# apache/auron

Measured on AMD Instinct MI355X. Metric: tpcds_suite_seconds, lower is better.
Workload: dtype decimal64/fp64

## Files before the change

auron_amd/config.py:

```python
from __future__ import annotations

import os
from dataclasses import dataclass
from typing import Any, Dict, Optional


@dataclass(frozen=True)
class ConfigOption:
    key: str
    default: Any
    typ: type
    doc: str = ""
    env: Optional[str] = None


_REGISTRY: Dict[str, ConfigOption] = {}


def _opt(key: str, default, typ, doc="", env=None) -> ConfigOption:
    o = ConfigOption(key, default, typ, doc, env)
    _REGISTRY[key] = o
    return o


BATCH_SIZE = _opt("spark.auron.batchSize", 1 << 22, int, "rows per in-flight batch")
MEMORY_FRACTION = _opt("spark.auron.memoryFraction", 0.8, float, "fraction of HBM the memmgr may use")
ENABLE_NATIVE = _opt("spark.auron.enable", True, bool, "master switch")
REQUIRE_NATIVE = _opt("spark.auron.requireNativeKernels", True, bool,
                      "fail loudly if HIP kernels missing on GPU", env="AURON_REQUIRE_NATIVE")
SPILL_COMPRESSION = _opt("spark.auron.spill.compression.codec", "lz4", str)
SHUFFLE_COMPRESSION = _opt("spark.auron.shuffle.compression.codec", "none", str,
                           "xGMI is fast enough that intra-node shuffle ships raw")
SMJ_FALLBACK_ENABLE = _opt("spark.auron.smjfallback.enable", False, bool, env="AURON_SMJ_FALLBACK")
SMJ_FALLBACK_ROWS = _opt("spark.auron.smjfallback.rows.threshold", 10_000_000, int, env="AURON_SMJ_FALLBACK_ROWS")
PARTIAL_AGG_SKIPPING_RATIO = _opt("spark.auron.partialAggSkipping.ratio", 0.999, float, env="AURON_PARTIAL_SKIP_RATIO")
UDF_FALLBACK = _opt("spark.auron.udf.hostFallback.enable", True, bool)
LOG_LEVEL = _opt("spark.auron.native.log.level", "WARN", str, env="AURON_LOG_LEVEL")
IGNORE_CORRUPTED_FILES = _opt("spark.auron.ignoreCorruptedFiles", False, bool,
                              "skip unreadable input files instead of failing the task",
                              env="AURON_IGNORE_CORRUPTED_FILES")
BROADCAST_MAX_ROWS = _opt("spark.auron.broadcast.maxRows", 20_000_000, int,
                          "estimated build-side rows above which the planner "
                          "shuffles both join sides instead of broadcasting",
                          env="AURON_BROADCAST_MAX_ROWS")
BROADCAST_CACHE_BYTES = _opt("spark.auron.broadcast.cache.maxBytes", 4 << 30, int,
                             "device bytes of build-once broadcast relations/"
                             "hash tables kept across queries",
                             env="AURON_BROADCAST_CACHE_BYTES")
FORCE_SHUFFLED_HASH_JOIN = _opt("spark.auron.forceShuffledHashJoin", False, bool,
                                "never broadcast: hash-exchange both sides",
                                env="AURON_FORCE_SHJ")
EXPR_FUSION = _opt("spark.auron.expr.fusion.enable", False, bool,
                   "compile project/filter scalar expression trees into one "
                   "fused interpreter kernel launch (k_expr_exec). Default "
                   "off: the kernel itself measures ~24us/launch but the "
                   "per-batch host dispatch costs more than the at::native "
                   "launches it replaces at TPC-DS shapes (same-box A/B: "
                   "SF=10 suite 8.24s on vs 6.52s off); worthwhile only for "
                   "very wide scalar-heavy projections until the native "
                   "plan walker absorbs the dispatch",
                   env="AURON_EXPR_FUSION")
AGG_STREAMING = _opt("spark.auron.agg.streaming.enable", True, bool,
                     "chunked spill-capable partial aggregation",
                     env="AURON_AGG_STREAMING")
HOST_SPILL_BUDGET = _opt("spark.auron.memory.hostSpillBudget", 64 << 30, int,
                         "host-DRAM bytes of spilled holders before the disk "
                         "tier engages", env="AURON_HOST_SPILL_BUDGET")
SHUFFLE_PERSIST = _opt("spark.auron.shuffle.persist", False, bool,
                       "route exchanges through durable .data/.index files "
                       "(stage-retry contract)", env="AURON_SHUFFLE_PERSIST")
PARQUET_NATIVE = _opt("spark.auron.parquet.native.enable", True, bool,
                      "device parquet decode (else pyarrow host read)",
                      env="AURON_PARQUET_NATIVE")
PARQUET_PAGE_DECOMPRESS = _opt("spark.auron.parquet.pageDecompression.enable",
                               True, bool,
                               "host-decompress snappy/zstd/gzip pages for "
                               "the device decode path")
PARTIAL_AGG_SKIPPING_MINROWS = _opt("spark.auron.partialAggSkipping.minRows",
                                    1 << 14, int,
                                    "below this many rows partial-agg "
                                    "skipping is never sampled")
SORT_LIMIT_TOPK = _opt("spark.auron.sort.topK.enable", True, bool,
                       "ORDER BY+LIMIT keeps only the top K rows per batch")
SORT_EXTERNAL_WIDE_KEYS = _opt("spark.auron.sort.external.wideKeys.enable",
                               True, bool,
                               "range-split external sort also for string and "
                               "decimal128 first keys (off: such sorts stay "
                               "monolithic and cannot spill)",
                               env="AURON_SORT_EXTERNAL_WIDE_KEYS")
EXCHANGE_SAMPLE_ROWS = _opt("spark.auron.rangePartition.sampleRows", 4096, int,
                            "per-rank sample size for range-partition bounds")
SCAN_CACHE_BYTES = _opt("spark.auron.scan.cache.maxBytes", 0, int,
                        "per-query decoded-scan cache budget; 0 = auto "
                        "(15% of HBM on GPU, 4 GB on CPU)",
                        env="AURON_SCAN_CACHE_BYTES")
STREAM_BYTES = _opt("spark.auron.stream.minInputBytes", -1, int,
                    "estimated agg-input bytes above which operators "
                    "stream instead of materializing; -1 = auto (8% of "
                    "HBM on GPU, 1 GB on CPU), 0 = always stream",
                    env="AURON_STREAM_BYTES")
SCAN_HBM_CACHE = _opt("spark.auron.scan.hbmStagedCache.maxBytes", 0, int,
                      "staged raw-page bytes kept device-resident across "
                      "reads; 0 = auto (30% of HBM)",
                      env="AURON_SCAN_HBM_CACHE")
HBM_CACHE_RESERVE = _opt("spark.auron.scan.hbmStagedCache.reserveFraction",
                         0.25, float,
                         "free-HBM fraction the staged-bytes cache must "
                         "never consume (evicts itself under pressure)")
SCAN_DELTA_NATIVE = _opt("spark.auron.scan.deltaNative.enable", True, bool,
                         "decode DELTA_BINARY_PACKED pages and "
                         "DELTA_LENGTH_BYTE_ARRAY / DELTA_BYTE_ARRAY string "
                         "pages with the k_pq_delta_* kernels from a "
                         "host-built miniblock index, DELTA_BYTE_ARRAY "
                         "strings rebuilt by k_pq_dba_bytes (off: "
                         "DELTA_BINARY_PACKED is expanded to PLAIN by one "
                         "host job per page and DELTA_LENGTH_BYTE_ARRAY and "
                         "DELTA_BYTE_ARRAY columns take the pyarrow host "
                         "read)",
                         env="AURON_SCAN_DELTA_NATIVE")
SCAN_PREFETCH = _opt("spark.auron.scan.streamPrefetch", 2, int,
                     "files decoded ahead of the consumer on the "
                     "streaming scan path")
SCAN_IO_THREADS = _opt("spark.auron.scan.ioThreads", 8, int,
                       "host page-read/staging thread-pool size",
                       env="AURON_SCAN_IO_THREADS")
STREAM_PEEK_FACTOR = _opt("spark.auron.stream.peekBatches", 8, int,
                          "batch-size multiples buffered before the "
                          "chunked agg commits to streaming")
STREAM_JOIN_PROBE = _opt("spark.auron.stream.joinProbe.enable", True, bool,
                         "probe build-right joins batch-by-batch on the "
                         "streaming path (GPU only)",
                         env="AURON_STREAM_JOIN_PROBE")
JOIN_FUSED_PROBE = _opt("spark.auron.join.fusedProbe.enable", True, bool,
                        "probe hash joins with the fused kernels "
                        "(k_join_probe_count / k_join_probe_fill / "
                        "k_join_exists: probe hash computed in-kernel, one "
                        "chain walk, per-tile offsets, key descriptors passed "
                        "by value) for up to 8 key columns (off: murmur3 + "
                        "k_join_count + torch scan + k_join_fill, and "
                        "join_counts for semi/anti/existence joins)",
                        env="AURON_JOIN_FUSED_PROBE")
DECIMAL128_NATIVE_ARITH = _opt("spark.auron.decimal128.nativeArith.enable",
                               True, bool,
                               "run exact decimal128 + - * /, comparisons, "
                               "casts, abs and CheckOverflow on the "
                               "k_dec128_* kernels (off: the exact "
                               "host-integer reference path, also on GPU "
                               "batches)",
                               env="AURON_DECIMAL128_NATIVE_ARITH")
SPILL_DIR = _opt("spark.auron.spill.dir", "", str,
                 "directory for disk-tier spill files (empty = system tmp)",
                 env="AURON_SPILL_DIR")
MEM_BUDGET = _opt("spark.auron.memory.budgetBytes", 0, int,
                  "absolute memmgr budget override; 0 = memoryFraction "
                  "of device/host memory", env="AURON_MEM_BUDGET")


class AuronConf:
    def __init__(self, overrides: Optional[Dict[str, Any]] = None):
        self._values: Dict[str, Any] = {}
        if overrides:
            for k, v in overrides.items():
                self.set(k, v)

    def set(self, key: str, value) -> "AuronConf":
        if key not in _REGISTRY:
            raise KeyError(f"unknown config {key}; known: {sorted(_REGISTRY)}")
        self._values[key] = value
        return self

    def get(self, opt: ConfigOption):
        if opt.key in self._values:
            return self._values[opt.key]
        if opt.env and opt.env in os.environ:
            raw = os.environ[opt.env]
            if opt.typ is bool:
                return raw not in ("0", "false", "False")
            return opt.typ(raw)
        return opt.default

    @staticmethod
    def options() -> Dict[str, ConfigOption]:
        return dict(_REGISTRY)
```

auron_amd/native/__init__.py:

```python
from __future__ import annotations

import ctypes
import os
from typing import List, Optional, Tuple

import numpy as np
import torch

_LIB_NAME = "libauron_hip.so"
_here = os.path.dirname(os.path.abspath(__file__))
LIB_PATH = os.path.join(_here, _LIB_NAME)

_lib = None
_load_error: Optional[str] = None


class AuronNativeMissing(RuntimeError):
    pass


def _try_load():
    global _lib, _load_error
    if _lib is not None or _load_error is not None:
        return
    if not os.path.exists(LIB_PATH):
        _load_error = f"{LIB_PATH} not built (run python -m auron_amd.native.build)"
        return
    try:
        lib = ctypes.CDLL(LIB_PATH)
    except OSError as e:
        _load_error = str(e)
        return
    c = ctypes.c_void_p
    i32 = ctypes.c_int32
    i64 = ctypes.c_int64
    lib.au_abi_version.restype = ctypes.c_int
    lib.au_murmur3.argtypes = [c, ctypes.c_int, i64, i32, c, c]
    lib.au_group_ids.argtypes = [c, ctypes.c_int, i64, c, i64, c, c, c, c, c, c]
    lib.au_join_build.argtypes = [i64, c, i64, c, c, c]
    lib.au_join_count.argtypes = [c, c, ctypes.c_int, i64, c, i64, c, c, c, c]
    lib.au_join_fill.argtypes = [c, c, ctypes.c_int, i64, c, i64, c, c, c, c, c, c, ctypes.c_int, c]
    lib.au_join_probe_tile.argtypes = []
    lib.au_join_probe_tile.restype = i64
    lib.au_join_probe_max_keys.argtypes = []
    lib.au_join_probe_max_keys.restype = ctypes.c_int
    lib.au_join_probe_count.argtypes = [c, ctypes.c_int, i64, c, i64, c, i32,
                                        ctypes.c_int, c, c, c, c, c]
    lib.au_join_probe_fill.argtypes = [c, ctypes.c_int, i64, c, c, c, c,
                                       ctypes.c_int, c, c, c]
    lib.au_join_exists.argtypes = [c, ctypes.c_int, i64, c, i64, c, i32, c, c]
    for f in ("au_join_probe_count", "au_join_probe_fill", "au_join_exists"):
        getattr(lib, f).restype = ctypes.c_int
    lib.au_pmod.argtypes = [c, i64, i32, c, c]
    lib.au_bytes_gather.argtypes = [c, c, c, c, i64, c]
    lib.au_multi_gather.argtypes = [c, i64, c, ctypes.c_int, c]
    lib.au_multi_gather.restype = ctypes.c_int
    lib.au_agg_scatter.argtypes = [c, i64, c, c, ctypes.c_int, ctypes.c_int,
                                   ctypes.c_int, c, c, i64, c]
    lib.au_agg_count.argtypes = [c, i64, c, c, c]
    lib.au_agg_multi.argtypes = [c, i64, c, ctypes.c_int, c]
    for f in ("au_agg_scatter", "au_agg_count", "au_agg_multi"):
        getattr(lib, f).restype = ctypes.c_int
    lib.au_pq_rle1.argtypes = [c, ctypes.c_int, c, c, c]
    lib.au_rle1_expand.argtypes = [c, i64, c, c, c]
    lib.au_rle1_expand.restype = ctypes.c_int
    lib.au_host_rle1_parse.argtypes = [c, i64, i64, i64, i64, c, i64]
    lib.au_host_rle1_parse.restype = i64
    lib.au_host_plainba_parse.argtypes = [c, i64, i64, c, c, i64]
    lib.au_host_plainba_parse.restype = i64
    lib.au_host_delta_unpack.argtypes = [c, i64, i64, i64, ctypes.c_int, c]
    lib.au_host_delta_unpack.restype = i64
    lib.au_host_delta_index.argtypes = [c, i64, i64, i64, i64, i64, i64, c, c,
                                        i64]
    lib.au_host_delta_index.restype = i64
    lib.au_pq_delta_sums.argtypes = [c, i64, c, c, c]
    lib.au_pq_delta_scan.argtypes = [c, i64, c]
    lib.au_pq_delta_emit.argtypes = [c, i64, c, i64, c, c, c, ctypes.c_int, c]
    for f in ("au_pq_delta_sums", "au_pq_delta_scan", "au_pq_delta_emit"):
        getattr(lib, f).restype = ctypes.c_int
    lib.au_host_dba_decode.argtypes = [c, i64, c, c, c, c, i64, c, i64]
    lib.au_host_dba_decode.restype = i64
    lib.au_pq_dba_tile.argtypes = []
    lib.au_pq_dba_tile.restype = i64
    lib.au_pq_dba_bytes.argtypes = [c, c, c, c, i64, i64, c, c, c]
    lib.au_pq_dba_bytes.restype = ctypes.c_int
    lib.au_pq_rle_idx.argtypes = [c, ctypes.c_int, c, c, c, c]
    lib.au_pq_scatter.argtypes = [c, ctypes.c_int, c, c, c, c, ctypes.c_int, i64, c]
    lib.au_pq_copy_plain.argtypes = [c, ctypes.c_int, c, c, ctypes.c_int, i64, c]
    for f in ("au_pq_rle1", "au_pq_rle_idx", "au_pq_scatter", "au_pq_copy_plain"):
        getattr(lib, f).restype = ctypes.c_int
    lib.au_expr_exec.argtypes = [c, ctypes.c_int, c, ctypes.c_int, c,
                                 ctypes.c_int, ctypes.c_int, i64, c]
    lib.au_expr_exec.restype = ctypes.c_int
    lib.au_part_hist.argtypes = [c, i64, i32, c, c]
    lib.au_part_scatter.argtypes = [c, i64, c, c, c, c]
    lib.au_range_bucket_str.argtypes = [c, c, i64, c, c, i32, ctypes.c_int, c, c]
    lib.au_range_bucket_i128.argtypes = [c, i64, c, i32, ctypes.c_int, c, c]
    for f in ("au_range_bucket_str", "au_range_bucket_i128"):
        getattr(lib, f).restype = ctypes.c_int
    f64 = ctypes.c_double
    lib.au_window_range_bounds_i64.argtypes = [c, c, c, i64, i64, i64,
                                               ctypes.c_int, c, c, c]
    lib.au_window_range_bounds_f64.argtypes = [c, c, c, i64, f64, f64,
                                               ctypes.c_int, c, c, c]
    lib.au_window_frame_minmax_i64.argtypes = [c, i64, c, i64, c, c, i64,
                                               ctypes.c_int, c, c]
    lib.au_window_frame_minmax_f64.argtypes = [c, i64, c, i64, c, c, i64,
                                               ctypes.c_int, c, c]
    lib.au_window_pyramid_size.argtypes = [i64]
    lib.au_window_pyramid_size.restype = i64
    lib.au_i128_scan_tile.argtypes = []
    lib.au_i128_scan_tile.restype = i64
    lib.au_prefix_sum_i128.argtypes = [c, c, i64, c, c, c]
    lib.au_window_frame_sum_i128.argtypes = [c, i64, c, c, i64, c, c]
    lib.au_window_frame_minmax_i128.argtypes = [c, i64, c, i64, c, c, i64,
                                                ctypes.c_int, c, c]
    for f in ("au_window_range_bounds_i64", "au_window_range_bounds_f64",
              "au_window_frame_minmax_i64", "au_window_frame_minmax_f64",
              "au_prefix_sum_i128", "au_window_frame_sum_i128",
              "au_window_frame_minmax_i128"):
        getattr(lib, f).restype = ctypes.c_int
    ci = ctypes.c_int
    u64 = ctypes.c_uint64
    lib.au_dec128_grid_threads.argtypes = []
    lib.au_dec128_grid_threads.restype = i64
    lib.au_dec128_addsub.argtypes = [c, ci, c, c, ci, c, i64, ci, ci, ci, ci,
                                     ci, c, c, c]
    lib.au_dec128_mul.argtypes = [c, ci, c, c, ci, c, i64, ci, ci, c, c, c]
    lib.au_dec128_div.argtypes = [c, ci, c, c, ci, c, i64, ci, ci, c, c, c]
    lib.au_dec128_cmp.argtypes = [c, ci, c, ci, i64, ci, ci, ci, c, c]
    lib.au_dec128_rescale.argtypes = [c, ci, c, i64, ci, ci, u64, u64, c, ci,
                                      c, c]
    for f in ("au_dec128_addsub", "au_dec128_mul", "au_dec128_div",
              "au_dec128_cmp", "au_dec128_rescale"):
        getattr(lib, f).restype = ctypes.c_int
    for f in ("au_murmur3", "au_group_ids", "au_join_build", "au_join_count",
              "au_join_fill", "au_pmod", "au_part_hist", "au_part_scatter"):
        getattr(lib, f).restype = ctypes.c_int
    _lib = lib


def available() -> bool:
    _try_load()
    return _lib is not None


def require():
    _try_load()
    if _lib is None:
        raise AuronNativeMissing(
            f"auron native HIP library unavailable: {_load_error}. "
            "Build it with `python -m auron_amd.native.build`."
        )
    return _lib


def lib():
    return require()


def host_lib():
    return require()


_DESC_DTYPE = np.dtype(
    [("data", "<u8"), ("offsets", "<u8"), ("validity", "<u8"),
     ("dtype", "<i4"), ("scale", "<i4")]
)
assert _DESC_DTYPE.itemsize == 32


def pack_descs_host(cols) -> Tuple[np.ndarray, list]:
    n = len(cols)
    arr = np.zeros(n, dtype=_DESC_DTYPE)
    keep = []
    for i, col in enumerate(cols):
        data = col.data
        if not data.is_contiguous():
            data = data.contiguous()
        if col.dtype.code == 12 and data.data_ptr() % 16:
            raise ValueError("decimal128 key column is not 16-byte aligned "
                             "(ops._key_cols aligns it)")
        keep.append(data)
        arr[i]["data"] = data.data_ptr()
        if col.offsets is not None:
            off = col.offsets.contiguous()
            keep.append(off)
            arr[i]["offsets"] = off.data_ptr()
        if col.validity is not None:
            v = col.validity.contiguous()
            keep.append(v)
# ... 25 lines not shown
```

auron_amd/native/csrc/kernels.hip:

```cpp

#include <hip/hip_runtime.h>
#include <stdint.h>

#define AU_EXPORT extern "C" __attribute__((visibility("default")))

enum AuDType : int32_t {
  AU_BOOL = 0,
  AU_INT8 = 1,
  AU_INT16 = 2,
  AU_INT32 = 3,
  AU_INT64 = 4,
  AU_FLOAT32 = 5,
  AU_FLOAT64 = 6,
  AU_DATE32 = 7,
  AU_STRING = 8,
  AU_DECIMAL64 = 9,
  AU_LIST = 10,
  AU_TIMESTAMP = 11,
  AU_DECIMAL128 = 12,
};

struct AuColDesc {
  const void* data;
  const int64_t* offsets;
// ... 120 lines not shown
      return hash_bytes((const uint8_t*)c.data + s, (int32_t)(e - s), seed);
    }
    case AU_DECIMAL128: {
      const ulonglong2 v = ((const ulonglong2*)c.data)[i];
      return hash_dec128(v.x, (int64_t)v.y, seed);
    }
  }
  return seed;
}

__global__ void k_murmur3(const AuColDesc* cols, int ncols, int64_t n,
                          uint32_t seed, int32_t* out) {
  for (int64_t i = (int64_t)blockIdx.x * blockDim.x + threadIdx.x; i < n;
       i += (int64_t)gridDim.x * blockDim.x) {
    uint32_t h = seed;
    for (int c = 0; c < ncols; c++) {
      if (row_valid(cols[c], i)) h = hash_one(cols[c], i, h);
    }
    out[i] = (int32_t)h;
  }
}

AU_EXPORT int au_murmur3(const void* cols_dev, int ncols, int64_t n,
                         int32_t seed, int32_t* out, void* stream) {
  if (n == 0) return 0;
  hipLaunchKernelGGL(k_murmur3, dim3(au_grid(n, 256)), dim3(256), 0,
                     (hipStream_t)stream, (const AuColDesc*)cols_dev, ncols, n,
                     (uint32_t)seed, out);
  return (int)hipGetLastError();
}

__device__ bool keys_equal(const AuColDesc* a_cols, int64_t ai,
                           const AuColDesc* b_cols, int64_t bi, int ncols) {
  for (int c = 0; c < ncols; c++) {
    const AuColDesc& a = a_cols[c];
    const AuColDesc& b = b_cols[c];
    bool av = row_valid(a, ai);
    bool bv = row_valid(b, bi);
    if (av != bv) return false;
    if (!av) continue;
    switch (a.dtype) {
      case AU_BOOL:
      case AU_INT8:
        if (((const int8_t*)a.data)[ai] != ((const int8_t*)b.data)[bi]) return false;
        break;
      case AU_INT16:
        if (((const int16_t*)a.data)[ai] != ((const int16_t*)b.data)[bi]) return false;
        break;
      case AU_INT32:
      case AU_DATE32:
        if (((const int32_t*)a.data)[ai] != ((const int32_t*)b.data)[bi]) return false;
        break;
      case AU_INT64:
      case AU_DECIMAL64:
      case AU_TIMESTAMP:
        if (((const int64_t*)a.data)[ai] != ((const int64_t*)b.data)[bi]) return false;
        break;
      case AU_FLOAT32:
        if (((const float*)a.data)[ai] != ((const float*)b.data)[bi]) return false;
        break;
      case AU_FLOAT64:
        if (((const double*)a.data)[ai] != ((const double*)b.data)[bi]) return false;
        break;
      case AU_STRING: {
        int64_t as = a.offsets[ai], ae = a.offsets[ai + 1];
        int64_t bs = b.offsets[bi], be = b.offsets[bi + 1];
        if (ae - as != be - bs) return false;
        const uint8_t* ap = (const uint8_t*)a.data + as;
        const uint8_t* bp = (const uint8_t*)b.data + bs;
        int32_t len = (int32_t)(ae - as);
        int32_t k = 0;
        for (; k + 8 <= len; k += 8) {
          uint64_t wa, wb;
          __builtin_memcpy(&wa, ap + k, 8);
          __builtin_memcpy(&wb, bp + k, 8);
          if (wa != wb) return false;
        }
        for (; k < len; k++)
          if (ap[k] != bp[k]) return false;
        break;
      }
      case AU_DECIMAL128: {
        const ulonglong2 va = ((const ulonglong2*)a.data)[ai];
        const ulonglong2 vb = ((const ulonglong2*)b.data)[bi];
        if (va.x != vb.x || va.y != vb.y) return false;
        break;
      }
    }
  }
  return true;
}

__global__ void k_group_insert(const AuColDesc* cols, int ncols, int64_t n,
                               int32_t* slots, uint32_t cap_mask,
                               const int32_t* hashes, int32_t* rep) {
  for (int64_t i = (int64_t)blockIdx.x * blockDim.x + threadIdx.x; i < n;
       i += (int64_t)gridDim.x * blockDim.x) {
    uint32_t p = ((uint32_t)hashes[i]) & cap_mask;
    int32_t me = (int32_t)i;
    while (true) {
      int32_t cur = slots[p];
      if (cur == -1) {
        int32_t prev = atomicCAS(&slots[p], -1, me);
        if (prev == -1) {
          rep[i] = me;
          break;
        }
        cur = prev;
      }
      if (keys_equal(cols, cur, cols, i, ncols)) {
        rep[i] = cur;
        break;
      }
      p = (p + 1) & cap_mask;
    }
  }
}

__global__ void k_group_assign(const int32_t* rep, int64_t n, int32_t* gid_of_row,
                               int64_t* rep_rows, int32_t* counter) {
  for (int64_t i = (int64_t)blockIdx.x * blockDim.x + threadIdx.x; i < n;
       i += (int64_t)gridDim.x * blockDim.x) {
    if (rep[i] == (int32_t)i) {
      int32_t g = atomicAdd(counter, 1);
      gid_of_row[i] = g;
      rep_rows[g] = i;
    }
  }
}

__global__ void k_group_gather(const int32_t* rep, int64_t n, int32_t* gid_of_row) {
  for (int64_t i = (int64_t)blockIdx.x * blockDim.x + threadIdx.x; i < n;
       i += (int64_t)gridDim.x * blockDim.x) {
    gid_of_row[i] = gid_of_row[rep[i]];
  }
}

AU_EXPORT int au_group_ids(const void* cols_dev, int ncols, int64_t n,
                           int32_t* slots, int64_t cap, const int32_t* hashes,
                           int32_t* rep, int32_t* gids, int64_t* rep_rows,
                           int32_t* counter, void* stream) {
  if (n == 0) return 0;
  hipStream_t s = (hipStream_t)stream;
  uint32_t mask = (uint32_t)(cap - 1);
  int g = au_grid(n, 256);
  hipLaunchKernelGGL(k_group_insert, dim3(g), dim3(256), 0, s,
                     (const AuColDesc*)cols_dev, ncols, n, slots, mask, hashes, rep);
  hipLaunchKernelGGL(k_group_assign, dim3(g), dim3(256), 0, s, rep, n, gids,
                     rep_rows, counter);
  hipLaunchKernelGGL(k_group_gather, dim3(g), dim3(256), 0, s, rep, n, gids);
  return (int)hipGetLastError();
}

__global__ void k_join_build(int64_t n, int32_t* heads, uint32_t cap_mask,
                             int32_t* next, const int32_t* hashes) {
  for (int64_t i = (int64_t)blockIdx.x * blockDim.x + threadIdx.x; i < n;
       i += (int64_t)gridDim.x * blockDim.x) {
    uint32_t p = ((uint32_t)hashes[i]) & cap_mask;
    next[i] = atomicExch(&heads[p], (int32_t)i);
  }
}

__device__ __forceinline__ bool join_row_has_null(const AuColDesc* cols,
                                                  int ncols, int64_t i) {
  for (int c = 0; c < ncols; c++)
    if (!row_valid(cols[c], i)) return true;
  return false;
}

__global__ void k_join_count(const AuColDesc* bcols, const AuColDesc* pcols,
                             int ncols, int64_t n_probe, const int32_t* heads,
                             uint32_t cap_mask, const int32_t* next,
                             const int32_t* phashes, int32_t* counts) {
  for (int64_t i = (int64_t)blockIdx.x * blockDim.x + threadIdx.x; i < n_probe;
       i += (int64_t)gridDim.x * blockDim.x) {
    int32_t cnt = 0;
    if (!join_row_has_null(pcols, ncols, i)) {
      int32_t j = heads[((uint32_t)phashes[i]) & cap_mask];
      while (j != -1) {
        if (keys_equal(bcols, j, pcols, i, ncols) &&
            !join_row_has_null(bcols, ncols, j))
          cnt++;
        j = next[j];
      }
    }
    counts[i] = cnt;
  }
}

__global__ void k_join_fill(const AuColDesc* bcols, const AuColDesc* pcols,
                            int ncols, int64_t n_probe, const int32_t* heads,
                            uint32_t cap_mask, const int32_t* next,
                            const int32_t* phashes, const int64_t* offsets,
                            int64_t* build_out, int64_t* probe_out,
                            uint8_t* build_matched, int emit_unmatched_probe) {
  for (int64_t i = (int64_t)blockIdx.x * blockDim.x + threadIdx.x; i < n_probe;
       i += (int64_t)gridDim.x * blockDim.x) {
    int64_t o = offsets[i];
    int64_t start = o;
    if (!join_row_has_null(pcols, ncols, i)) {
      int32_t j = heads[((uint32_t)phashes[i]) & cap_mask];
      while (j != -1) {
        if (keys_equal(bcols, j, pcols, i, ncols) &&
            !join_row_has_null(bcols, ncols, j)) {
          build_out[o] = j;
          probe_out[o] = i;
          if (build_matched) build_matched[j] = 1;
          o++;
        }
        j = next[j];
      }
    }
    if (emit_unmatched_probe && o == start) {
      build_out[o] = -1;
      probe_out[o] = i;
    }
  }
}

AU_EXPORT int au_join_build(int64_t n, int32_t* heads, int64_t cap,
                            int32_t* next, const int32_t* hashes, void* stream) {
  if (n == 0) return 0;
  hipLaunchKernelGGL(k_join_build, dim3(au_grid(n, 256)), dim3(256), 0,
                     (hipStream_t)stream, n, heads, (uint32_t)(cap - 1), next,
                     hashes);
  return (int)hipGetLastError();
}

AU_EXPORT int au_join_count(const void* bcols, const void* pcols, int ncols,
                            int64_t n_probe, const int32_t* heads, int64_t cap,
                            const int32_t* next, const int32_t* phashes,
                            int32_t* counts, void* stream) {
  if (n_probe == 0) return 0;
  hipLaunchKernelGGL(k_join_count, dim3(au_grid(n_probe, 256)), dim3(256), 0,
                     (hipStream_t)stream, (const AuColDesc*)bcols,
                     (const AuColDesc*)pcols, ncols, n_probe, heads,
                     (uint32_t)(cap - 1), next, phashes, counts);
  return (int)hipGetLastError();
}

AU_EXPORT int au_join_fill(const void* bcols, const void* pcols, int ncols,
                           int64_t n_probe, const int32_t* heads, int64_t cap,
                           const int32_t* next, const int32_t* phashes,
                           const int64_t* offsets, int64_t* build_out,
                           int64_t* probe_out, uint8_t* build_matched,
                           int emit_unmatched_probe, void* stream) {
  if (n_probe == 0) return 0;
  hipLaunchKernelGGL(k_join_fill, dim3(au_grid(n_probe, 256)), dim3(256), 0,
                     (hipStream_t)stream, (const AuColDesc*)bcols,
                     (const AuColDesc*)pcols, ncols, n_probe, heads,
                     (uint32_t)(cap - 1), next, phashes, offsets, build_out,
                     probe_out, build_matched, emit_unmatched_probe);
  return (int)hipGetLastError();
}

#define JP_MAX_KEYS 8
#define JP_BLOCK 256
#define JP_SLABS 4
#define JP_TILE (JP_BLOCK * JP_SLABS)

struct JpKeys {
  AuColDesc build[JP_MAX_KEYS];
  AuColDesc probe[JP_MAX_KEYS];
};

template <int MODE>
__device__ __forceinline__ bool jp_probe_key(const JpKeys& k, int ncols,
                                             int64_t i, int64_t* pkey) {
  if (MODE == 0) return !join_row_has_null(k.probe, ncols, i);
  const uint8_t* v = k.probe[0].validity;
  if (v != nullptr && v[i] == 0) return false;
  if (MODE == 1) *pkey = ((const int64_t*)k.probe[0].data)[i];
  else *pkey = ((const int32_t*)k.probe[0].data)[i];
  return true;
}

template <int MODE>
__device__ __forceinline__ uint32_t jp_hash(const JpKeys& k, int ncols,
                                            int64_t i, int64_t pkey,
                                            uint32_t seed) {
  if (MODE == 1) return hash_long((uint64_t)pkey, seed);
  if (MODE == 2) return hash_int((uint32_t)(int32_t)pkey, seed);
  uint32_t h = seed;
  for (int c = 0; c < ncols; c++) h = hash_one(k.probe[c], i, h);
  return h;
}

template <int MODE>
__device__ __forceinline__ bool jp_match(const JpKeys& k, int ncols, int32_t j,
                                         int64_t i, int64_t pkey) {
  if (MODE == 0)
    return keys_equal(k.build, j, k.probe, i, ncols) &&
           !join_row_has_null(k.build, ncols, j);
  const uint8_t* v = k.build[0].validity;
  if (MODE == 1) {
    if (((const int64_t*)k.build[0].data)[j] != pkey) return false;
  } else {
    if (((const int32_t*)k.build[0].data)[j] != (int32_t)pkey) return false;
  }
  return v == nullptr || v[j] != 0;
}

template <int MODE>
__global__ void __launch_bounds__(JP_BLOCK) k_join_probe_count(
    JpKeys k, int ncols, int64_t n_probe, int64_t n_tiles,
    const int32_t* __restrict__ heads, uint32_t cap_mask,
// ... 364 lines not shown
```

auron_amd/ops.py:

```python
from __future__ import annotations

import os
from typing import List, Optional, Tuple

import torch

from . import dtypes, native
from .column import Column

SPARK_SEED = 42
_M32 = 0xFFFFFFFF
_M64 = (1 << 64) - 1


def _use_native(device: torch.device) -> bool:
    if device.type != "cuda":
        return False
    if os.environ.get("AURON_FORCE_REF", "0") == "1":
        return False
    if os.environ.get("AURON_REQUIRE_NATIVE", "1") == "0" and not native.available():
        return False
    native.require()
    return True

# ... 68 lines not shown
    idx = skip[:, None] + torch.arange(16, device=d.device)[None, :]
    return _hash_padded_bytes_t(B.gather(1, idx.clamp(max=15)), lens, 16, h)


def _spark_narrow_decimal(dt) -> bool:
    return dt.code == dtypes.DECIMAL128 and dt.precision <= 18


def murmur3_ref(cols: List[Column], seed: int = SPARK_SEED) -> torch.Tensor:
    n = len(cols[0])
    device = cols[0].device
    h = torch.full((n,), seed, dtype=torch.int64, device=device)
    for c in cols:
        if c.dtype.is_string:
            from . import strings as S

            lens = S.lengths(c)
            maxlen = int(lens.max().item()) if n else 0
            padded = S.to_padded(c, max(maxlen, 1)).to(torch.int64)
            hv = _hash_padded_bytes_t(padded, lens, maxlen, h)
        else:
            d = c.data
            code = c.dtype.code
            if code in (dtypes.BOOL,):
                v = d.to(torch.int64)
                hv = _hash_int_t(v, h)
            elif code in (dtypes.INT8, dtypes.INT16, dtypes.INT32, dtypes.DATE32):
                v = d.to(torch.int64) & _M32
                hv = _hash_int_t(v, h)
            elif code in (dtypes.INT64, dtypes.DECIMAL64):
                v = d.to(torch.int64)
                hv = _hash_long_t(v, h)
            elif code == dtypes.FLOAT32:
                f = torch.where(d == 0, torch.zeros_like(d), d)
                v = f.view(torch.int32).to(torch.int64) & _M32
                hv = _hash_int_t(v, h)
            elif code == dtypes.FLOAT64:
                f = torch.where(d == 0, torch.zeros_like(d), d)
                v = f.view(torch.int64)
                hv = _hash_long_t(v, h)
            elif code == dtypes.DECIMAL128:
                if _spark_narrow_decimal(c.dtype):
                    hv = _hash_long_t(d[:, 0], h)
                else:
                    hv = _hash_dec128_t(d, h)
            else:
                raise TypeError(c.dtype.name)
        if c.validity is not None:
            h = torch.where(c.validity, hv, h)
        else:
            h = hv
    h = torch.where(h >= 2 ** 31, h - 2 ** 32, h)
    return h.to(torch.int32)


def _key_cols(cols: List[Column]) -> List[Column]:
    out = []
    for c in cols:
        if c.dtype.code == dtypes.DECIMAL128:
            d = _i128_aligned(c.data)
            if d is not c.data:
                c = Column(c.dtype, d, c.validity)
        out.append(c)
    return out


def _spark_hash_cols(cols: List[Column]) -> List[Column]:
    out = []
    for c in cols:
        if _spark_narrow_decimal(c.dtype):
            c = Column(dtypes.decimal64(c.dtype.precision, c.dtype.scale),
                       c.data[:, 0].contiguous(), c.validity)
        out.append(c)
    return out


def _murmur3_native(cols: List[Column], seed: int = SPARK_SEED) -> torch.Tensor:
    device = cols[0].device
    n = len(cols[0])
    lib = native.lib()
    out = torch.empty(n, dtype=torch.int32, device=device)
    descs, keep = native.pack_descs(_key_cols(cols), device)
    rc = lib.au_murmur3(descs.data_ptr(), len(cols), n, seed, out.data_ptr(),
                        native.stream_ptr(device))
    native.check(rc, "au_murmur3")
    del keep
    return out


def murmur3(cols: List[Column], seed: int = SPARK_SEED) -> torch.Tensor:
    device = cols[0].device
    if not _use_native(device):
        return murmur3_ref(cols, seed)
    return _murmur3_native(_spark_hash_cols(cols), seed)


def _join_hash(cols: List[Column]) -> torch.Tensor:
    return _murmur3_native(cols)


def _next_pow2(x: int) -> int:
    p = 1024
    while p < x:
        p <<= 1
    return p


def _key_tuple_lists(cols: List[Column]):
    import math

    lists = []
    for c in cols:
        if c.dtype.code == dtypes.DECIMAL128:
            d = c.data.to("cpu")
            valid = None if c.validity is None else c.validity.tolist()
            vals = [(h << 64) | (l & _M64) for l, h in
                    zip(d[:, 0].tolist(), d[:, 1].tolist())]
            if valid is not None:
                vals = [v if ok else None for v, ok in zip(vals, valid)]
            lists.append(vals)
            continue
        vals = c.to_pylist()
        if c.dtype.is_float:
            vals = ["NaN" if (v is not None and isinstance(v, float) and math.isnan(v)) else v for v in vals]
        lists.append(vals)
    return list(zip(*lists)) if cols else []


def group_ids_ref(cols: List[Column]) -> Tuple[torch.Tensor, torch.Tensor]:
    keys = _key_tuple_lists(cols)
    d = {}
    gids = []
    reps = []
    for i, k in enumerate(keys):
        g = d.get(k)
        if g is None:
            g = len(d)
            d[k] = g
            reps.append(i)
        gids.append(g)
    device = cols[0].device
    return (torch.tensor(gids, dtype=torch.int64, device=device),
            torch.tensor(reps, dtype=torch.int64, device=device))


def group_ids(cols: List[Column]) -> Tuple[torch.Tensor, torch.Tensor]:
    device = cols[0].device
    n = len(cols[0])
    if n == 0:
        return (torch.empty(0, dtype=torch.int64, device=device),
                torch.empty(0, dtype=torch.int64, device=device))
    if not _use_native(device):
        return group_ids_ref(cols)
    lib = native.lib()
    cols = _key_cols(cols)
    hashes = murmur3(cols)
    cap = _next_pow2(2 * n)
    slots = torch.full((cap,), -1, dtype=torch.int32, device=device)
    rep = torch.empty(n, dtype=torch.int32, device=device)
    gids = torch.empty(n, dtype=torch.int32, device=device)
    rep_rows = torch.empty(n, dtype=torch.int64, device=device)
    counter = torch.zeros(1, dtype=torch.int32, device=device)
    descs, keep = native.pack_descs(cols, device)
    rc = lib.au_group_ids(descs.data_ptr(), len(cols), n, slots.data_ptr(), cap,
                          hashes.data_ptr(), rep.data_ptr(), gids.data_ptr(),
                          rep_rows.data_ptr(), counter.data_ptr(),
                          native.stream_ptr(device))
    native.check(rc, "au_group_ids")
    ng = int(counter.item())
    del keep
    return gids.to(torch.int64), rep_rows[:ng]


def hash_join_ref(build_cols, probe_cols, emit_unmatched_probe, need_build_matched):
    bkeys = _key_tuple_lists(build_cols)
    pkeys = _key_tuple_lists(probe_cols)
    table = {}
    for j, k in enumerate(bkeys):
        if any(v is None for v in k):
            continue
        table.setdefault(k, []).append(j)
    n_build = len(build_cols[0]) if build_cols else 0
    matched = [False] * n_build
    bi, pi = [], []
    for i, k in enumerate(pkeys):
        rows = [] if any(v is None for v in k) else table.get(k, [])
        if rows:
            for j in rows:
                bi.append(j)
                pi.append(i)
                matched[j] = True
        elif emit_unmatched_probe:
            bi.append(-1)
            pi.append(i)
    device = probe_cols[0].device
    bm = torch.tensor(matched, dtype=torch.bool, device=device) if need_build_matched else None
    return (torch.tensor(bi, dtype=torch.int64, device=device),
            torch.tensor(pi, dtype=torch.int64, device=device), bm)



class JoinTable:

    __slots__ = ("heads", "nxt", "cap", "bhash", "n_build")

    def __init__(self, heads, nxt, cap, bhash, n_build):
        self.heads = heads
        self.nxt = nxt
        self.cap = cap
        self.bhash = bhash
        self.n_build = n_build

    @property
    def nbytes(self):
        return (self.heads.numel() + self.nxt.numel()) * 4 + self.bhash.numel() * 8


def join_build(build_cols: List[Column]) -> Optional["JoinTable"]:
    device = build_cols[0].device
    if not _use_native(device):
        return None
    lib = native.lib()
    sp = native.stream_ptr(device)
    n_build = len(build_cols[0])
    bhash = _join_hash(build_cols)
    cap = _next_pow2(2 * max(n_build, 1))
    heads = torch.full((cap,), -1, dtype=torch.int32, device=device)
    nxt = torch.empty(max(n_build, 1), dtype=torch.int32, device=device)
    if n_build:
        rc = lib.au_join_build(n_build, heads.data_ptr(), cap, nxt.data_ptr(),
                               bhash.data_ptr(), sp)
        native.check(rc, "au_join_build")
    return JoinTable(heads, nxt, cap, bhash, n_build)


JOIN_PROBE_MAX_KEYS = 8


def _fused_probe_enabled() -> bool:
    from .config import JOIN_FUSED_PROBE, AuronConf

    return bool(AuronConf().get(JOIN_FUSED_PROBE))


def join_probe_tile() -> int:
    return int(native.lib().au_join_probe_tile())


def _join_key_descs(build_cols, probe_cols):
    import numpy as np

    barr, bkeep = native.pack_descs_host(_key_cols(build_cols))
    parr, pkeep = native.pack_descs_host(_key_cols(probe_cols))
    return np.concatenate([barr, parr]), (bkeep, pkeep)


def hash_join(build_cols: List[Column], probe_cols: List[Column],
              emit_unmatched_probe: bool = False,
              need_build_matched: bool = False,
              table: Optional["JoinTable"] = None):
    device = probe_cols[0].device
    n_probe = len(probe_cols[0])
    n_build = len(build_cols[0])
    if not _use_native(device):
        return hash_join_ref(build_cols, probe_cols, emit_unmatched_probe, need_build_matched)
    if table is None:
        table = join_build(build_cols)
    if len(build_cols) <= JOIN_PROBE_MAX_KEYS and _fused_probe_enabled():
        return _hash_join_fused(build_cols, probe_cols, emit_unmatched_probe,
                                need_build_matched, table)
    return _hash_join_legacy(build_cols, probe_cols, emit_unmatched_probe,
                             need_build_matched, table)


def _hash_join_fused(build_cols, probe_cols, emit_unmatched_probe,
                     need_build_matched, table):
    device = probe_cols[0].device
    n_probe = len(probe_cols[0])
    n_build = len(build_cols[0])
    lib = native.lib()
    sp = native.stream_ptr(device)
    bm = torch.zeros(n_build, dtype=torch.uint8, device=device) if need_build_matched else None
    if n_probe == 0:
        empty = torch.empty(0, dtype=torch.int64, device=device)
        return empty, empty.clone(), (bm.bool() if bm is not None else None)
    ncols = len(build_cols)
    descs, keep = _join_key_descs(build_cols, probe_cols)
    tile = join_probe_tile()
    n_tiles = (n_probe + tile - 1) // tile
    counts = torch.empty(n_probe, dtype=torch.int32, device=device)
    first = torch.empty(n_probe, dtype=torch.int32, device=device)
    tile_sums = torch.empty(n_tiles, dtype=torch.int64, device=device)
    emit = 1 if emit_unmatched_probe else 0
    rc = lib.au_join_probe_count(descs.ctypes.data, ncols, n_probe,
                                 table.heads.data_ptr(), table.cap,
                                 table.nxt.data_ptr(), SPARK_SEED, emit,
                                 counts.data_ptr(), first.data_ptr(),
                                 tile_sums.data_ptr(),
                                 bm.data_ptr() if bm is not None and n_build else None,
                                 sp)
    native.check(rc, "au_join_probe_count")
    tile_ends = torch.cumsum(tile_sums, 0)
    total = int(tile_ends[-1].item())
    build_idx = torch.empty(max(total, 1), dtype=torch.int64, device=device)
    probe_idx = torch.empty(max(total, 1), dtype=torch.int64, device=device)
    rc = lib.au_join_probe_fill(descs.ctypes.data, ncols, n_probe,
# ... 1047 lines not shown
```

Baseline: 2.887.

## Fuse group-id assignment into a single hash-build kernel with in-kernel hashing

Replaces the murmur3 + insert + assign + gather + int32→int64 copy sequence for GROUP BY ids with one kernel, k_group_build. It computes the row hash in-kernel, takes key descriptors by value, and numbers each group by the row that wins its slot, using one atomic per block tile. A small finish kernel then writes the int64 ids. There are specialised single-int64 and single-int32 key paths. The aim is to cut kernel launches, descriptor uploads and intermediate memory passes. In exchange it adds a probe-overflow check and a host sync on a two-element counter.

```diff
diff --git a/auron_amd/config.py b/auron_amd/config.py
--- a/auron_amd/config.py
+++ b/auron_amd/config.py
@@ -140,6 +140,16 @@
                         "k_join_count + torch scan + k_join_fill, and "
                         "join_counts for semi/anti/existence joins)",
                         env="AURON_JOIN_FUSED_PROBE")
+AGG_FUSED_GROUP_IDS = _opt("spark.auron.agg.fusedGroupIds.enable", True, bool,
+                           "assign GROUP BY / DISTINCT / partition ids with "
+                           "the fused kernels (k_group_build: row hash "
+                           "computed in-kernel, key descriptors passed by "
+                           "value, a group numbered by the row that wins its "
+                           "slot with one atomic per wave; k_group_finish "
+                           "writes int64 ids) for up to 16 key columns (off: "
+                           "murmur3 + k_group_insert + k_group_assign + "
+                           "k_group_gather + an int32 -> int64 copy)",
+                           env="AURON_AGG_FUSED_GROUP_IDS")
 DECIMAL128_NATIVE_ARITH = _opt("spark.auron.decimal128.nativeArith.enable",
                                True, bool,
                                "run exact decimal128 + - * /, comparisons, "
diff --git a/auron_amd/native/__init__.py b/auron_amd/native/__init__.py
--- a/auron_amd/native/__init__.py
+++ b/auron_amd/native/__init__.py
@@ -37,6 +37,13 @@
     lib.au_abi_version.restype = ctypes.c_int
     lib.au_murmur3.argtypes = [c, ctypes.c_int, i64, i32, c, c]
     lib.au_group_ids.argtypes = [c, ctypes.c_int, i64, c, i64, c, c, c, c, c, c]
+    lib.au_group_max_keys.argtypes = []
+    lib.au_group_max_keys.restype = ctypes.c_int
+    lib.au_group_tile.argtypes = []
+    lib.au_group_tile.restype = i64
+    lib.au_group_ids_fused.argtypes = [c, ctypes.c_int, i64, c, i64, i32, c, c,
+                                       c, c, c]
+    lib.au_group_ids_fused.restype = ctypes.c_int
     lib.au_join_build.argtypes = [i64, c, i64, c, c, c]
     lib.au_join_count.argtypes = [c, c, ctypes.c_int, i64, c, i64, c, c, c, c]
     lib.au_join_fill.argtypes = [c, c, ctypes.c_int, i64, c, i64, c, c, c, c, c, c, ctypes.c_int, c]
diff --git a/auron_amd/native/csrc/kernels.hip b/auron_amd/native/csrc/kernels.hip
--- a/auron_amd/native/csrc/kernels.hip
+++ b/auron_amd/native/csrc/kernels.hip
@@ -296,6 +296,299 @@
   return (int)hipGetLastError();
 }
 
+#define GK_MAX_KEYS 16
+#define GK_BLOCK 256
+#define GK_SLABS 4
+#define GK_TILE (GK_BLOCK * GK_SLABS)
+#define GK_GROUP 4
+
+struct GkKeys {
+  AuColDesc c[GK_MAX_KEYS];
+};
+
+struct __attribute__((aligned(8))) GkPair {
+  uint64_t x, y;
+};
+
+__device__ __forceinline__ int gk_wshift(int32_t dtype) {
+  return (int)((0x4333323232100ull >> (4 * dtype)) & 15);
+}
+
+__device__ __forceinline__ const GkPair* gk_addr(const AuColDesc& c, int64_t i) {
+  const bool str = c.dtype == AU_STRING;
+  const char* base = str ? (const char*)c.offsets : (const char*)c.data;
+  const char* p = base + (i << gk_wshift(c.dtype));
+  return (const GkPair*)(p - (str ? 0 : (uintptr_t)p & 15));
+}
+
+__device__ __forceinline__ uint64_t gk_fixed(const AuColDesc& c, int64_t i,
+                                             GkPair q) {
+  const int sh = gk_wshift(c.dtype);
+  const uint32_t off =
+      ((uint32_t)(uintptr_t)c.data + ((uint32_t)i << sh)) & 15u;
+  uint64_t v = (off & 8u) ? q.y : q.x;
+  v >>= (off & 7u) * 8u;
+  if (sh < 3) v &= (1ull << (8u << sh)) - 1ull;
+  return v;
+}
+
+__device__ __forceinline__ bool gk_same(const AuColDesc& c, int64_t a,
+                                        int64_t b, GkPair qa, GkPair qb) {
+  uint64_t a0 = qa.x, a1 = qa.y, b0 = qb.x, b1 = qb.y;
+  if (c.dtype != AU_STRING && c.dtype != AU_DECIMAL128) {
+    a0 = gk_fixed(c, a, qa);
+    b0 = gk_fixed(c, b, qb);
+  }
+  switch (c.dtype) {
+    case AU_FLOAT32:
+      return !(__uint_as_float((uint32_t)a0) != __uint_as_float((uint32_t)b0));
+    case AU_FLOAT64:
+      return !(__longlong_as_double((long long)a0) !=
+               __longlong_as_double((long long)b0));
+    case AU_STRING: {
+      if (a1 - a0 != b1 - b0) return false;
+      const uint8_t* ap = (const uint8_t*)c.data + a0;
+      const uint8_t* bp = (const uint8_t*)c.data + b0;
+      const int32_t len = (int32_t)(a1 - a0);
+      bool same = true;
+      int32_t k = 0;
+      for (; same && k + 8 <= len; k += 8) {
+        uint64_t wa, wb;
+        __builtin_memcpy(&wa, ap + k, 8);
+        __builtin_memcpy(&wb, bp + k, 8);
+        same = wa == wb;
+      }
+      for (; same && k < len; k++) same = ap[k] == bp[k];
+      return same;
+    }
+    case AU_DECIMAL128:
+      return a0 == b0 && a1 == b1;
+    default:
+      return a0 == b0;
+  }
+}
+
+__device__ __forceinline__ bool gk_equal(const GkKeys& k, int ncols, int64_t a,
+                                         int64_t b, const uint8_t* mapped) {
+  bool eq = true;
+#pragma unroll 1
+  for (int c0 = 0; eq && c0 < ncols; c0 += GK_GROUP) {
+    GkPair qa[GK_GROUP], qb[GK_GROUP];
+    uint8_t va[GK_GROUP], vb[GK_GROUP];
+#pragma unroll
+    for (int u = 0; u < GK_GROUP; u++) {
+      const AuColDesc& c = k.c[c0 + u < ncols ? c0 + u : ncols - 1];
+      const uint8_t* v = c.validity;
+      va[u] = *(v != nullptr ? v + a : mapped);
+      vb[u] = *(v != nullptr ? v + b : mapped);
+      qa[u] = *gk_addr(c, a);
+      qb[u] = *gk_addr(c, b);
+    }
+#pragma unroll
+    for (int u = 0; u < GK_GROUP; u++) {
+      if (eq && c0 + u < ncols) {
+        const AuColDesc& c = k.c[c0 + u];
+        const bool av = c.validity == nullptr || va[u] != 0;
+        const bool bv = c.validity == nullptr || vb[u] != 0;
+        if (av != bv) eq = false;
+        else if (av) eq = gk_same(c, a, b, qa[u], qb[u]);
+      }
+    }
+  }
+  return eq;
+}
+
+template <int MODE>
+__device__ __forceinline__ uint32_t gk_hash(const GkKeys& k, int ncols,
+                                            int64_t i, uint32_t seed,
+                                            int64_t* own, bool* own_valid) {
+  if (MODE == 0) {
+    uint32_t h = seed;
+    for (int c = 0; c < ncols; c++)
+      if (row_valid(k.c[c], i)) h = hash_one(k.c[c], i, h);
+    return h;
+  }
+  const uint8_t* v = k.c[0].validity;
+  *own_valid = v == nullptr || v[i] != 0;
+  if (MODE == 1) {
+    *own = ((const int64_t*)k.c[0].data)[i];
+    return *own_valid ? hash_long((uint64_t)*own, seed) : seed;
+  }
+  *own = ((const int32_t*)k.c[0].data)[i];
+  return *own_valid ? hash_int((uint32_t)(int32_t)*own, seed) : seed;
+}
+
+template <int MODE>
+__device__ __forceinline__ bool gk_match(const GkKeys& k, int ncols,
+                                         int32_t cur, int64_t i, int64_t own,
+                                         bool own_valid,
+                                         const uint8_t* mapped) {
+  if (MODE == 0) return gk_equal(k, ncols, cur, i, mapped);
+  const uint8_t* v = k.c[0].validity;
+  const bool cv = v == nullptr || v[cur] != 0;
+  const int64_t x = MODE == 1 ? ((const int64_t*)k.c[0].data)[cur]
+                              : (int64_t)((const int32_t*)k.c[0].data)[cur];
+  return cv == own_valid && (!own_valid || x == own);
+}
+
+template <int MODE>
+__global__ void __launch_bounds__(GK_BLOCK) k_group_build(
+    GkKeys k, int ncols, int64_t n, int64_t n_tiles, int32_t* slots,
+    uint32_t cap_mask, uint32_t seed, int32_t* __restrict__ tmp,
+    int64_t* __restrict__ rep_rows, int32_t* counter) {
+  const int tid = threadIdx.x;
+  const int lane = tid & 63, wave = tid >> 6;
+  __shared__ int32_t wtot[GK_BLOCK / 64];
+  __shared__ int32_t tile_g0;
+  for (int64_t t = blockIdx.x; t < n_tiles; t += gridDim.x) {
+    const int64_t base = t * GK_TILE;
+    uint32_t won = 0;
+    uint32_t p0[GK_SLABS];
+    int32_t cur0[GK_SLABS];
+    int64_t own[GK_SLABS];
+    bool ownv[GK_SLABS];
+#pragma unroll
+    for (int s = 0; s < GK_SLABS; s++) {
+      p0[s] = 0;
+      own[s] = 0;
+      ownv[s] = true;
+    }
+    if (MODE == 0) {
+#pragma unroll 1
+      for (int s = 0; s < GK_SLABS; s++) {
+        const int64_t i = base + s * GK_BLOCK + tid;
+        uint32_t h = 0;
+        if (i < n) h = gk_hash<MODE>(k, ncols, i, seed, &own[0], &ownv[0]) & cap_mask;
+#pragma unroll
+        for (int u = 0; u < GK_SLABS; u++)
+          if (s == u) p0[u] = h;
+      }
+    } else {
+#pragma unroll
+      for (int s = 0; s < GK_SLABS; s++) {
+        const int64_t i = base + s * GK_BLOCK + tid;
+        if (i < n)
+          p0[s] = gk_hash<MODE>(k, ncols, i, seed, &own[s], &ownv[s]) & cap_mask;
+      }
+    }
+#pragma unroll
+    for (int s = 0; s < GK_SLABS; s++) {
+      const int64_t i = base + s * GK_BLOCK + tid;
+      cur0[s] = i < n ? slots[p0[s]] : -1;
+    }
+#pragma unroll 1
+    for (int s = 0; s < GK_SLABS; s++) {
+      const int64_t i = base + s * GK_BLOCK + tid;
+      bool active = i < n;
+      uint32_t p = p0[0];
+      int32_t cur = cur0[0];
+      int64_t okey = own[0];
+      bool okv = ownv[0];
+#pragma unroll
+      for (int u = 1; u < GK_SLABS; u++) {
+        if (s == u) {
+          p = p0[u];
+          cur = cur0[u];
+          okey = own[u];
+          okv = ownv[u];
+        }
+      }
+      uint32_t visited = 0;
+      while (active) {
+        if (cur == -1) {
+          const int32_t prev = atomicCAS(&slots[p], -1, (int32_t)i);
+          if (prev == -1) {
+            won |= 1u << s;
+            break;
+          }
+          cur = prev;
+        }
+        if (gk_match<MODE>(k, ncols, cur, i, okey, okv,
+                           (const uint8_t*)slots)) {
+          tmp[i] = cur;
+          active = false;
+        } else if (++visited > cap_mask) {
+          counter[1] = 1;
+          active = false;
+        } else {
+          p = (p + 1) & cap_mask;
+          cur = slots[p];
+        }
+      }
+    }
+    const int32_t cnt = __popc(won);
+    int32_t incl = cnt;
+    for (int d = 1; d < 64; d <<= 1) {
+      const int32_t up = __shfl_up(incl, d, 64);
+      if (lane >= d) incl += up;
+    }
+    if (lane == 63) wtot[wave] = incl;
+    __syncthreads();
+    if (tid == 0) {
+      int32_t total = 0;
+      for (int w = 0; w < GK_BLOCK / 64; w++) total += wtot[w];
+      tile_g0 = total ? atomicAdd(&counter[0], total) : 0;
+    }
+    __syncthreads();
+    int32_t g = tile_g0 + incl - cnt;
+    for (int w = 0; w < wave; w++) g += wtot[w];
+#pragma unroll
+    for (int s = 0; s < GK_SLABS; s++) {
+      if (won & (1u << s)) {
+        const int64_t i = base + s * GK_BLOCK + tid;
+        rep_rows[g] = i;
+        tmp[i] = -1 - g;
+        g++;
+      }
+    }
+    __syncthreads();
+  }
+}
+
+__global__ void __launch_bounds__(GK_BLOCK) k_group_finish(
+    const int32_t* __restrict__ tmp, int64_t n, int64_t* __restrict__ gids) {
+  for (int64_t i = (int64_t)blockIdx.x * blockDim.x + threadIdx.x; i < n;
+       i += (int64_t)gridDim.x * blockDim.x) {
+    const int32_t v = tmp[i];
+    gids[i] = v < 0 ? -1 - v : -1 - tmp[v];
+  }
+}
+
+AU_EXPORT int au_group_max_keys() { return GK_MAX_KEYS; }
+AU_EXPORT int64_t au_group_tile() { return GK_TILE; }
+
+AU_EXPORT int au_group_ids_fused(const void* host_descs, int ncols, int64_t n,
+                                 int32_t* slots, int64_t cap, int32_t seed,
+                                 int32_t* tmp, int64_t* gids, int64_t* rep_rows,
+                                 int32_t* counter, void* stream) {
+  if (n == 0) return 0;
+  if (ncols < 1 || ncols > GK_MAX_KEYS) return 1002;
+  if (n > 0x7fffffffLL || cap < n || (cap & (cap - 1)) != 0) return 1003;
+  const AuColDesc* d = (const AuColDesc*)host_descs;
+  GkKeys k{};
+  for (int c = 0; c < ncols; c++) k.c[c] = d[c];
+  int mode = 0;
+  if (ncols == 1) {
+    const int32_t t = d[0].dtype;
+    if (t == AU_INT64 || t == AU_DECIMAL64 || t == AU_TIMESTAMP) mode = 1;
+    else if (t == AU_INT32 || t == AU_DATE32) mode = 2;
+  }
+  hipStream_t s = (hipStream_t)stream;
+  const int64_t n_tiles = (n + GK_TILE - 1) / GK_TILE;
+  const int grid = (int)(n_tiles > 2048 ? 2048 : n_tiles);
+#define GK_LAUNCH_BUILD(M)                                                    \
+  hipLaunchKernelGGL(k_group_build<M>, dim3(grid), dim3(GK_BLOCK), 0, s, k,   \
+                     ncols, n, n_tiles, slots, (uint32_t)(cap - 1),           \
+                     (uint32_t)seed, tmp, rep_rows, counter)
+  if (mode == 1) GK_LAUNCH_BUILD(1);
+  else if (mode == 2) GK_LAUNCH_BUILD(2);
+  else GK_LAUNCH_BUILD(0);
+#undef GK_LAUNCH_BUILD
+  hipLaunchKernelGGL(k_group_finish, dim3(au_grid(n, GK_BLOCK)), dim3(GK_BLOCK),
+                     0, s, tmp, n, gids);
+  return (int)hipGetLastError();
+}
+
 __global__ void k_join_build(int64_t n, int32_t* heads, uint32_t cap_mask,
                              int32_t* next, const int32_t* hashes) {
   for (int64_t i = (int64_t)blockIdx.x * blockDim.x + threadIdx.x; i < n;
diff --git a/auron_amd/ops.py b/auron_amd/ops.py
--- a/auron_amd/ops.py
+++ b/auron_amd/ops.py
@@ -244,6 +244,52 @@
                 torch.empty(0, dtype=torch.int64, device=device))
     if not _use_native(device):
         return group_ids_ref(cols)
+    if len(cols) <= GROUP_MAX_KEYS and _fused_group_ids_enabled():
+        return _group_ids_fused(cols)
+    return _group_ids_legacy(cols)
+
+
+GROUP_MAX_KEYS = 16
+
+
+def _fused_group_ids_enabled() -> bool:
+    from .config import AGG_FUSED_GROUP_IDS, AuronConf
+
+    return bool(AuronConf().get(AGG_FUSED_GROUP_IDS))
+
+
+def group_ids_tile() -> int:
+    return int(native.lib().au_group_tile())
+
+
+def _group_ids_fused(cols: List[Column]) -> Tuple[torch.Tensor, torch.Tensor]:
+    device = cols[0].device
+    n = len(cols[0])
+    lib = native.lib()
+    cap = _next_pow2(2 * n)
+    slots = torch.full((cap,), -1, dtype=torch.int32, device=device)
+    tmp = torch.empty(n, dtype=torch.int32, device=device)
+    gids = torch.empty(n, dtype=torch.int64, device=device)
+    rep_rows = torch.empty(n, dtype=torch.int64, device=device)
+    counter = torch.zeros(2, dtype=torch.int32, device=device)
+    descs, keep = native.pack_descs_host(_key_cols(cols))
+    rc = lib.au_group_ids_fused(descs.ctypes.data, len(cols), n,
+                                slots.data_ptr(), cap, SPARK_SEED,
+                                tmp.data_ptr(), gids.data_ptr(),
+                                rep_rows.data_ptr(), counter.data_ptr(),
+                                native.stream_ptr(device))
+    native.check(rc, "au_group_ids_fused")
+    ng, overflow = counter.tolist()
+    del keep
+    if overflow:
+        raise RuntimeError(f"au_group_ids_fused: a row visited all {cap} slots "
+                           f"of the group table ({n} rows)")
+    return gids, rep_rows[:ng]
+
+
+def _group_ids_legacy(cols: List[Column]) -> Tuple[torch.Tensor, torch.Tensor]:
+    device = cols[0].device
+    n = len(cols[0])
     lib = native.lib()
     cols = _key_cols(cols)
     hashes = murmur3(cols)
diff --git a/profiles/measure_group_ids.py b/profiles/measure_group_ids.py
--- /dev/null
+++ b/profiles/measure_group_ids.py
@@ -0,0 +1,133 @@
+import argparse
+import json
+import os
+import statistics
+import sys
+
+import torch
+
+sys.path.insert(0, os.path.join(os.path.dirname(os.path.abspath(__file__)), ".."))
+from auron_amd import dtypes, native, ops
+from auron_amd.column import Column
+
+DEV = "cuda:0"
+ENV = "AURON_AGG_FUSED_GROUP_IDS"
+INFINITY_CACHE = 256 << 20
+
+
+def _int_col(v, dt=dtypes.int64, valid=None):
+    return Column(dt, v.to(DEV).to(dt.torch_dtype), valid, None)
+
+
+def _str_col(v, valid=None):
+    v = v.to(DEV)
+    n = v.numel()
+    mat = torch.full((n, 20), ord("x"), dtype=torch.uint8, device=DEV)
+    q = v.clone()
+    for j in range(8):
+        mat[:, j] = (q % 26 + ord("a")).to(torch.uint8)
+        q //= 26
+    lens = 10 + v % 11
+    keep = torch.arange(20, device=DEV)[None, :] < lens[:, None]
+    offs = torch.zeros(n + 1, dtype=torch.int64, device=DEV)
+    torch.cumsum(lens, 0, out=offs[1:])
+    return Column(dtypes.string, mat[keep], valid, offs)
+
+
+def _timed(fn, warm, reps):
+    out, ts = {}, {"0": [], "1": []}
+    for s in ("0", "1"):
+        os.environ[ENV] = s
+        for _ in range(warm):
+            out[s] = fn()
+    torch.cuda.synchronize()
+    for _ in range(reps):
+        for s in ("0", "1"):
+            os.environ[ENV] = s
+            e0 = torch.cuda.Event(enable_timing=True)
+            e1 = torch.cuda.Event(enable_timing=True)
+            e0.record()
+            out[s] = fn()
+            e1.record()
+            torch.cuda.synchronize()
+            ts[s].append(e0.elapsed_time(e1))
+    os.environ.pop(ENV, None)
+
+    def stat(v):
+        return {"median": round(statistics.median(v), 4), "min": round(min(v), 4),
+                "max": round(max(v), 4)}
+
+    return out["0"], out["1"], stat(ts["0"]), stat(ts["1"])
+
+
+def _same_partition(a, b):
+    (ga, ra), (gb, rb) = a, b
+    g = ra.numel()
+    if g != rb.numel() or ga.dtype != torch.int64 or gb.dtype != torch.int64:
+        return False
+    to_b = gb[ra]
+    return bool(torch.equal(torch.sort(to_b).values, torch.arange(g, device=DEV))
+                and torch.equal(to_b[ga], gb))
+
+
+def _bytes(cols, n):
+    b = 0
+    for c in cols:
+        b += c.data.numel() * c.data.element_size()
+        if c.offsets is not None:
+            b += c.offsets.numel() * 8
+        if c.validity is not None:
+            b += c.validity.numel()
+    cap = ops._next_pow2(2 * n)
+    return b + cap * 4 + n * (4 + 8 + 8)
+
+
+def main():
+    ap = argparse.ArgumentParser()
+    ap.add_argument("--rows", type=int, default=16_000_000)
+    ap.add_argument("--reps", type=int, default=20)
+    args = ap.parse_args()
+    assert torch.cuda.is_available(), "needs a GPU"
+    native.require()
+    n = args.rows
+    g = torch.Generator().manual_seed(0)
+
+    def case(name, cols):
+        off, on, t_off, t_on = _timed(lambda: ops.group_ids(cols), 3, args.reps)
+        touched = _bytes(cols, n)
+        print(json.dumps({"case": name, "rows": n, "key_columns": len(cols),
+                          "groups": int(on[1].numel()),
+                          "same_partition": _same_partition(off, on),
+                          "touched_mb": round(touched / 2 ** 20, 1),
+                          "fits_infinity_cache": touched <= INFINITY_CACHE,
+                          "legacy_ms": t_off, "fused_ms": t_on,
+                          "speedup_median": round(t_off["median"] / t_on["median"], 3)}),
+              flush=True)
+
+    case("one int64 key, 1000 groups",
+         [_int_col(torch.randint(0, 1000, (n,), generator=g) * 7919)])
+    case("one int64 key, 4M groups",
+         [_int_col(torch.randint(0, 4_000_000, (n,), generator=g) * 7919)])
+
+    gid = torch.randint(0, 1_000_000, (n,), generator=g)
+    case("three strings (10-20 B) + int32, 1M groups",
+         [_str_col(gid), _str_col(gid * 7 + 1), _str_col(gid % 1000),
+          _int_col(1998 + gid % 4, dtypes.int32)])
+
+    gid = torch.randint(0, 1_000_000, (n,), generator=g)
+    level = (torch.arange(n) % 3).to(DEV)
+    live = [level < 3 - (1 if c >= 1 else 0) - (1 if c >= 4 else 0) for c in range(8)]
+    keys = [_str_col(gid % 50), _str_col(gid % 1000, live[1]),
+            _int_col(gid % 7, valid=live[2]), _str_col(gid // 1000, live[3]),
+            _int_col(2000 + gid % 3, dtypes.int32, live[4]), _str_col(gid, live[5]),
+            _int_col(gid % 12, dtypes.int32, live[6]), _str_col(gid * 3 + 2, live[7]),
+            _int_col(torch.tensor([0, 15, 127])[level.cpu()])]
+    case("nine keys (five strings, three ints, grouping id), a third NULL-filled", keys)
+    del keys, live
+
+    case("one int64 key, all rows distinct",
+         [_int_col(torch.randperm(n, generator=g) * 7919)])
+
+
+if __name__ == "__main__":
+    main()
diff --git a/profiles/trace_suite.py b/profiles/trace_suite.py
--- /dev/null
+++ b/profiles/trace_suite.py
@@ -0,0 +1,113 @@
+import argparse
+import csv
+import glob
+import json
+import os
+import statistics
+import sys
+
+MARKER = "FillFunctor<c10::Half>"
+WATCH = ["k_group_insert", "k_group_assign", "k_group_gather", "k_group_build<0>",
+         "k_group_build<1>", "k_group_build<2>", "k_group_finish", "k_murmur3",
+         "direct_copy", "FillFunctor<int>", "__amd_rocclr_copyBuffer"]
+
+
+def run(args):
+    import shutil
+
+    import torch
+
+    sys.path.insert(0, os.path.join(os.path.dirname(os.path.abspath(__file__)), ".."))
+    from auron_amd import AuronSession
+    from auron_amd.tpcds import datagen
+    from auron_amd.tpcds.queries import QUERIES, Catalog
+
+    root = args.data_root
+    if not root:
+        root = os.path.join(os.path.dirname(os.path.abspath(__file__)), "..", "data")
+        shm = "/dev/shm"
+        if os.path.isdir(shm) and os.access(shm, os.W_OK) and \
+                shutil.disk_usage(shm).free > shutil.disk_usage(os.path.dirname(root)).free:
+            root = os.path.join(shm, "auron_tpcds")
+    datagen.write_dataset(root, args.sf, rank=0, world=1)
+    session = AuronSession(device="cuda")
+    cat = Catalog(root, args.sf)
+
+    def marker():
+        torch.cuda.synchronize()
+        torch.empty(3, dtype=torch.float16, device="cuda").fill_(1)
+        torch.cuda.synchronize()
+
+    for _ in range(args.passes):
+        marker()
+        for qn in sorted(QUERIES):
+            session.collect(QUERIES[qn](cat, session))
+    marker()
+
+
+def stats(args):
+    paths = glob.glob(os.path.join(args.dir, "**", "*kernel_trace.csv"), recursive=True)
+    assert len(paths) == 1, paths
+    rows = []
+    with open(paths[0], newline="") as f:
+        for r in csv.DictReader(f):
+            rows.append((int(r["Start_Timestamp"]), int(r["End_Timestamp"]), r["Kernel_Name"]))
+    rows.sort()
+    passes, cur = [], None
+    for start, end, name in rows:
+        if MARKER in name:
+            if cur:
+                passes.append(cur)
+            cur = []
+        elif cur is not None:
+            cur.append((name, end - start))
+    assert passes, "no marker kernels in the trace"
+
+    def watch_key(name):
+        for w in WATCH:
+            if w in name and (w != "direct_copy" or "{lambda(long)#1}" in name):
+                return w
+        return None
+
+    summary = []
+    for p in passes:
+        w = {}
+        for name, d in p:
+            k = watch_key(name)
+            if k:
+                c = w.setdefault(k, [0, 0])
+                c[0] += 1
+                c[1] += d
+        summary.append({"launches": len(p), "kernel_ms": round(sum(d for _, d in p) / 1e6, 3),
+                        "watch": {k: [c, round(t / 1e6, 3)] for k, (c, t) in sorted(w.items())}})
+    per = {}
+    for name, d in passes[-1]:
+        per.setdefault(name, []).append(d)
+    total = sum(sum(v) for v in per.values())
+    with open(args.out, "w", newline="") as f:
+        wr = csv.writer(f, quoting=csv.QUOTE_NONNUMERIC)
+        wr.writerow(["Name", "Calls", "TotalDurationNs", "AverageNs", "Percentage",
+                     "MinNs", "MaxNs", "StdDev"])
+        for name, v in sorted(per.items(), key=lambda kv: -sum(kv[1])):
+            wr.writerow([name, len(v), sum(v), round(sum(v) / len(v), 6),
+                         round(100.0 * sum(v) / total, 4), min(v), max(v),
+                         round(statistics.pstdev(v), 6)])
+    print(json.dumps({"trace": os.path.basename(args.out), "passes": summary}), flush=True)
+
+
+def main():
+    ap = argparse.ArgumentParser()
+    sub = ap.add_subparsers(dest="cmd", required=True)
+    r = sub.add_parser("run")
+    r.add_argument("--sf", type=float, default=10.0)
+    r.add_argument("--passes", type=int, default=3)
+    r.add_argument("--data-root", type=str, default=os.environ.get("AURON_DATA_ROOT", ""))
+    s = sub.add_parser("stats")
+    s.add_argument("dir")
+    s.add_argument("out")
+    a = ap.parse_args()
+    run(a) if a.cmd == "run" else stats(a)
+
+
+if __name__ == "__main__":
+    main()
```

Result: slower. 3.063 (+6.1%).
